# luisdiaz1997/GPzoo

Measured on AMD Instinct MI355X. Metric: ELBO evals/sec (L=32-latent evaluations, all GPUs) at M=2048 inducing, N=200000, L=32 latents/GPU x 1 GPU(s), higher is better.
Workload: dtype f32; 1 GPU; BASELINE configs[2]: Slide-seq-shaped synthetic, N=200000 spots, M=2048, L=32 latents/GPU x 1 GPU(s), matern32, f32; latents_total=32, whitened=True, chunk=0, factor_dtype=f64

## Files before the change

gpzoo_amd/csrc/gemmw.hip:

```cpp
#include "gemmw.h"

#include "cov.h"


#include <cmath>
#include <mutex>
#include <type_traits>
#include <utility>

#ifndef GPZ_W_ABL
#define GPZ_W_ABL 0
#endif

namespace gpz {

typedef float f32x4 __attribute__((ext_vector_type(4)));

enum { WB_MEM = 0, WB_GEN = 1 };
enum { WA_DENSE = 0, WA_LOWER = 1, WA_UPPER = 2 };
enum { WE_STORE_STATS = 0,
       WE_STATS = 1,
       WE_STORE = 2,
       WE_STORE_COLSCALE = 3,
       WE_WBAR = 4,
       WE_KBAR = 5,
       WE_ADD_COLSCALE = 6 };

struct WParams {
  const float* A; int64_t lda, sA0;
  const float* B; int64_t ldb, sB0;
  const float* Z; int64_t MD;
  const float* X; int64_t nreal;
  const float* sigma; const float* ell;
  float* C; int64_t ldc, sC0;
  const float* mu; int64_t sMu;
  float* ps_sq; float* ps_mu; int64_t ncols;
  const float* colscale; const float* colvec; int64_t sCs;
  const float* rowvec; int64_t sRv;
  const float* aux;
  int64_t M;
  int L, nblk, mtw, nt, W, strips;
  int pair, colmajor;
  const int32_t* gate;
};

constexpr int W_BK = 16;

template <int TM, int TN, int BSRC, int D>
struct WLds {
  static constexpr int A_ELEMS = TM * W_BK;
  static constexpr int RPP = 256 / TN;
  static constexpr int PITCH = 256 + (RPP == 2 ? 8 : RPP == 1 ? 4 : 16);
  static constexpr int B_ELEMS = (W_BK / RPP) * PITCH;
  static constexpr int STAGE = A_ELEMS + B_ELEMS;
  static constexpr int ZB = 128 * D;
  static constexpr size_t bytes = sizeof(float) * (2 * STAGE + (BSRC == WB_GEN ? 2 * ZB : 0));
};

template <int TM, int TN, int BSRC, int ATRI, int EPI, int KIND, int D>
__global__ __launch_bounds__(64 * (TM / 128) * (TN / 32)) __attribute__((amdgpu_waves_per_eu(4, 4))) void gemmw_kernel(const WParams p) {
  constexpr int BK = W_BK;
  if (p.gate && *p.gate == 0) return;
  constexpr int WMW = TM / 128, WNW = TN / 32;
  constexpr int NW = WMW * WNW;
  static_assert(NW == 8 || NW == 16, "8 or 16 waves of 128 x 32");
  using G = WLds<TM, TN, BSRC, D>;
  constexpr int RPP = G::RPP, PITCH = G::PITCH;
  extern __shared__ __attribute__((aligned(1024))) char smem_raw[];
  float* const smem = reinterpret_cast<float*>(smem_raw);
  auto sA = [&](int buf) -> float* { return smem + buf * G::STAGE; };
  auto sB = [&](int buf) -> float* { return smem + buf * G::STAGE + G::A_ELEMS; };
  float* const sZ = smem + 2 * G::STAGE;
  auto addrB = [](int k, int n) { return (k / RPP) * PITCH + (k % RPP) * TN + n; };

  int tj, b0, leg_ti[2], nlegs = 1;
  {
    const int bid = blockIdx.x;
    const int x = bid & 7, s = bid >> 3;
    if (BSRC == WB_GEN) {
      const int ug = s / p.W, within = s - ug * p.W;
      const int u = ug * 8 + x;
      const int per_level = p.L * p.strips;
      if (u >= p.mtw * per_level) return;
      const int level = u / per_level, rem = u - level * per_level;
      leg_ti[0] = leg_ti[1] = (ATRI == WA_LOWER) ? p.mtw - 1 - level : level;
      b0 = rem / p.strips;
      tj = (rem - b0 * p.strips) * p.W + within;
    } else {
      const int per_unit = (p.pair ? (p.mtw + 1) >> 1 : p.mtw) * p.W;
      const int u = (s / per_unit) * 8 + x, within = s % per_unit;
      if (u >= p.L * p.strips) return;
      b0 = u / p.strips;
      const int nrow = p.pair ? (p.mtw + 1) >> 1 : p.mtw;
      const int pi = p.colmajor ? within % nrow : within / p.W, far = p.pair ? p.mtw - 1 - pi : pi;
      const int strip = u - b0 * p.strips, c0 = strip * p.nt / p.strips, c1 = (strip + 1) * p.nt / p.strips;
      tj = c0 + (p.colmajor ? within / nrow : within % p.W);
      if (tj >= c1) return;
      const bool long_first = ((s >> 5) & 1) == 0;
      leg_ti[0] = ((ATRI == WA_LOWER) == long_first) ? far : pi;
      leg_ti[1] = ((ATRI == WA_LOWER) == long_first) ? pi : far;
      nlegs = far == pi ? 1 : 2;
      if (!p.pair) leg_ti[0] = leg_ti[1] = (ATRI == WA_LOWER) ? p.mtw - 1 - pi : pi;
    }
    if (tj >= p.nt) return;
  }
  const int tid = threadIdx.x, lane = tid & 63;
  const int wave = __builtin_amdgcn_readfirstlane(tid >> 6);
  const int wn = wave % WNW;
  const int r = lane & 15, q = lane >> 4;
  const int Mp = p.nblk * 128;

  typedef __attribute__((address_space(3))) void lds_void;
  constexpr int NPA = TM / (16 * NW);
#if defined(__HIP_DEVICE_COMPILE__)
  const __amdgpu_buffer_rsrc_t a_rsrc = __builtin_amdgcn_make_buffer_rsrc(
      const_cast<float*>(p.A + b0 * p.sA0), 0, (int)(p.lda * Mp * sizeof(float)), 0x00020000);
  const __amdgpu_buffer_rsrc_t b_rsrc = __builtin_amdgcn_make_buffer_rsrc(
      const_cast<float*>(BSRC == WB_MEM ? p.B + b0 * p.sB0 : p.Z), 0,
      (int)((BSRC == WB_MEM ? p.ldb * Mp : p.MD) * sizeof(float)), 0x00020000);
#endif
  auto k_begin_of = [&](int ti) { return (ATRI == WA_UPPER) ? TM * ti : 0; };
  auto k_end_of = [&](int ti) { return (ATRI == WA_LOWER) ? min(TM * (ti + 1), Mp) : Mp; };
  int a_soff[NPA], b_soff = 0;
  auto gperm = [](int w) { const int t = (w >> 2) & 3; return (((t >> 1) ^ t) & 1) << 1 | (t >> 1); };
  const int a_voff = ((lane >> 2) * (int)p.lda + (((lane & 3) ^ gperm(lane >> 2)) * 4)) * (int)sizeof(float);
  const int b_voff = ((lane / (TN / 4)) * (int)p.ldb + (lane % (TN / 4)) * 4) * (int)sizeof(float);
  bool abl_first = true;
  auto stage_load = [&](int buf) __attribute__((always_inline)) {
    if ((GPZ_W_ABL & 2) && !abl_first) return;
    abl_first = false;
#if defined(__HIP_DEVICE_COMPILE__)
#pragma unroll
    for (int h = 0; h < NPA; ++h) {
      __builtin_amdgcn_raw_ptr_buffer_load_lds(a_rsrc, (lds_void*)(sA(buf) + (NPA * wave + h) * 256), 16, a_voff, a_soff[h], 0, 0);
      a_soff[h] += BK * (int)sizeof(float);
    }
    if constexpr (BSRC == WB_MEM) {
      constexpr int NPB = (W_BK / RPP) / NW;
      static_assert(BSRC != WB_MEM || (NPB * NW * RPP == W_BK && NPB >= 1), "whole B pieces per wave");
#pragma unroll
      for (int h = 0; h < NPB; ++h)
        __builtin_amdgcn_raw_ptr_buffer_load_lds(b_rsrc, (lds_void*)(sB(buf) + (wave + NW * h) * PITCH), 16, b_voff,
                                                 b_soff + h * NW * RPP * (int)p.ldb * (int)sizeof(float), 0, 0);
      b_soff += BK * (int)p.ldb * (int)sizeof(float);
    }
#endif
  };
  auto tile_begin = [&](int ti) __attribute__((always_inline)) {
    const int kb = k_begin_of(ti);
#pragma unroll
    for (int h = 0; h < NPA; ++h) {
      int row = ti * TM + (NPA * wave + h) * 16;
      while (row >= Mp) row -= 128;
      a_soff[h] = (row * (int)p.lda + kb) * (int)sizeof(float);
    }
    b_soff = ((kb + RPP * wave) * (int)p.ldb + tj * TN) * (int)sizeof(float);
    stage_load(0);
  };

  constexpr int NXC = TN / 64;
  float xc[NXC][D], ampn[NXC], c0n[NXC], c2n[NXC];
  CovConst cc = {0.f, 0.f, 0.f, 0.f};
  if constexpr (BSRC == WB_GEN) {
    cc = cov_const<KIND>(p.sigma[b0], p.ell[b0]);
#pragma unroll
    for (int h = 0; h < NXC; ++h) {
      const int64_t n = (int64_t)tj * TN + h * 64 + lane;
      const bool real = n < p.nreal;
#pragma unroll
      for (int k = 0; k < D; ++k) xc[h][k] = real ? p.X[n * D + k] : 0.f;
      ampn[h] = real ? cc.amp : 0.f;
      c0n[h] = (KIND != 0 && !real) ? 0.f : cc.c0;
      c2n[h] = real ? cc.c2 : 0.f;
    }
  }
  auto z_load = [&](int blk) __attribute__((always_inline)) {
#if defined(__HIP_DEVICE_COMPILE__)
    if (wave < 2 * D)
      __builtin_amdgcn_raw_ptr_buffer_load_lds(b_rsrc, (lds_void*)(sZ + (blk & 1) * G::ZB + wave * 64), 4, lane * 4,
                                               (blk * G::ZB + wave * 64) * 4, 0, 0);
#endif
  };
  auto b_generate = [&](int buf, int step) __attribute__((always_inline)) {
#pragma unroll
    for (int i = 0; i < BK / NW; ++i) {
      const int kk = wave + NW * i, kg = step * BK + kk;
      const float* zp = sZ + ((kg >> 7) & 1) * G::ZB + (kg & 127) * D;
      float z[D];
#pragma unroll
      for (int k = 0; k < D; ++k) z[k] = zp[k];
#pragma unroll
      for (int h = 0; h < NXC; ++h) {
        const float v = (GPZ_W_ABL & 1) ? z[0] + xc[h][0]
                                        : cov_value<KIND>(cov_radial<KIND>(cov_d2<D>(z, xc[h])), ampn[h], c0n[h], cc.c1, c2n[h]);
        sB(buf)[addrB(kk, h * 64 + lane)] = v;
      }
    }
  };

  f32x4 acc[8][2];

  int wm = 0, nk = 0, db = 0, n_a = 0, fr_a = 0, step0 = 0, t = 0, next_ti = -1;
  bool active = false;
  int fr_b[4];
#pragma unroll
  for (int j = 0; j < 4; ++j) fr_b[j] = addrB(4 * q + j, wn * 32 + r);

  auto mma_step = [&](int buf, auto lo_c, auto hi_c) __attribute__((always_inline)) {
    constexpr int LO = decltype(lo_c)::value, HI = decltype(hi_c)::value;
    float bf[4][2];
#pragma unroll
    for (int j = 0; j < 4; ++j)
#pragma unroll
      for (int ni = 0; ni < 2; ++ni) bf[j][ni] = sB(buf)[fr_b[j] + ni * 16];
#pragma unroll
    for (int half = 0; half < 2; ++half) {
      f32x4 fa[4];
#pragma unroll
      for (int m = 0; m < 4; ++m)
        if (half * 4 + m >= LO && half * 4 + m <= HI)
          fa[m] = *reinterpret_cast<const f32x4*>(sA(buf) + fr_a + (half * 4 + m) * 16 * BK);
#pragma unroll
      for (int j = 0; j < 4; ++j)
#pragma unroll
        for (int m = 0; m < 4; ++m)
#pragma unroll
          for (int ni = 0; ni < 2; ++ni)
            if (half * 4 + m >= LO && half * 4 + m <= HI)
              acc[half * 4 + m][ni] = __builtin_amdgcn_mfma_f32_16x16x4f32(fa[m][j], bf[j][ni], acc[half * 4 + m][ni], 0, 0, 0);
    }
  };

  using std::integral_constant;
  auto step = [&](auto par_c, auto run_c, auto lo_c, auto hi_c) __attribute__((always_inline)) {
    constexpr int P = decltype(par_c)::value;
    if (t + 1 < nk) {
      stage_load(P ^ 1);
      if constexpr (BSRC == WB_GEN) {
        const int st = step0 + t;
        if ((st & 7) == 0 && (st >> 3) + 1 < p.nblk) z_load((st >> 3) + 1);
        b_generate(P ^ 1, st + 1);
      }
    } else if (next_ti >= 0) {
      tile_begin(next_ti);
    }
    if constexpr (decltype(run_c)::value) mma_step(P, lo_c, hi_c);
    if (GPZ_W_ABL & 16) {
      asm volatile("s_waitcnt lgkmcnt(0)" ::: "memory");
      __builtin_amdgcn_s_barrier();
    } else {
      asm volatile("s_waitcnt vmcnt(0)" ::: "memory");
      if (!(GPZ_W_ABL & 8)) __syncthreads();
    }
    ++t;
  };
  using no_run = integral_constant<bool, false>;
  using run = integral_constant<bool, true>;
  using i0 = integral_constant<int, 0>;
  using i1 = integral_constant<int, 1>;
  using i7 = integral_constant<int, 7>;
  auto idle_until = [&](int end) __attribute__((always_inline)) {
    while (t < end) { step(i0{}, no_run{}, i0{}, i7{}); step(i1{}, no_run{}, i0{}, i7{}); }
  };
  auto full_until = [&](int end) __attribute__((always_inline)) {
    while (t < end) { step(i0{}, run{}, i0{}, i7{}); step(i1{}, run{}, i0{}, i7{}); }
  };
  auto diagonal = [&](auto self, auto u_c) __attribute__((always_inline)) -> void {
    constexpr int U = decltype(u_c)::value;
    if constexpr (ATRI == WA_LOWER) step(integral_constant<int, U & 1>{}, run{}, integral_constant<int, U>{}, i7{});
    else step(integral_constant<int, U & 1>{}, run{}, i0{}, integral_constant<int, U>{});
    if constexpr (U + 1 < 8) self(self, integral_constant<int, U + 1>{});
  };

  tile_begin(leg_ti[0]);
#pragma unroll 1
  for (int leg = 0; leg < nlegs; ++leg) {
    const int ti = leg_ti[leg];
    wm = WMW == 1 ? 0 : (wave / WNW) ^ ((ti ^ tj) & 1);
    const int k_begin = k_begin_of(ti);
    nk = (k_end_of(ti) - k_begin) / BK;
    db = WMW * ti + wm;
    active = db < p.nblk && (int64_t)tj * TN + wn * 32 < p.ncols;
    n_a = 8 * (ATRI == WA_LOWER ? db : wm);
    fr_a = (wm * 128 + r) * BK + ((q ^ gperm(r)) * 4);
    step0 = k_begin / BK;
    t = 0;
    next_ti = leg + 1 < nlegs ? leg_ti[leg + 1] : -1;
#pragma unroll
    for (int mi = 0; mi < 8; ++mi)
#pragma unroll
      for (int ni = 0; ni < 2; ++ni) acc[mi][ni] = f32x4{0, 0, 0, 0};
    if constexpr (BSRC == WB_GEN) {
      z_load(step0 >> 3);
      asm volatile("s_waitcnt vmcnt(0)" ::: "memory");
      __syncthreads();
      b_generate(0, step0);
    }
    if (leg == 0) asm volatile("s_waitcnt vmcnt(0)" ::: "memory");
    asm volatile("s_waitcnt lgkmcnt(0)" ::: "memory");
    __builtin_amdgcn_s_barrier();
    if (!active) {
      idle_until(nk);
    } else if constexpr (ATRI == WA_DENSE) {
      full_until(nk);
    } else if constexpr (ATRI == WA_LOWER) {
      full_until(n_a);
      diagonal(diagonal, i0{});
      idle_until(nk);
    } else {
      idle_until(n_a);
      diagonal(diagonal, i0{});
      full_until(nk);
    }

    if (!active) continue;
    if (GPZ_W_ABL & 4) {
      float sum = 0.f;
#pragma unroll
      for (int mi = 0; mi < 8; ++mi)
#pragma unroll
        for (int ni = 0; ni < 2; ++ni)
#pragma unroll
          for (int g = 0; g < 4; ++g) sum += acc[mi][ni][g];
      if (sum == 12345.678f) p.ps_sq[0] = sum;
      continue;
    }
    const int64_t row0 = (int64_t)db * 128;
    const int64_t ccol0 = (int64_t)tj * TN + wn * 32;
    if (BSRC == WB_GEN && row0 + 128 > p.M) {
#pragma unroll
      for (int mi = 0; mi < 8; ++mi)
#pragma unroll
        for (int g = 0; g < 4; ++g)
          if (row0 + mi * 16 + 4 * q + g >= p.M) {
#pragma unroll
            for (int ni = 0; ni < 2; ++ni) acc[mi][ni][g] = 0.f;
          }
    }
    if constexpr (EPI == WE_STORE_STATS || EPI == WE_STATS) {
      float ssq[2] = {0.f, 0.f}, smu[2] = {0.f, 0.f};
#pragma unroll
      for (int mi = 0; mi < 8; ++mi) {
        f32x4 m4 = {0, 0, 0, 0};
        if constexpr (EPI == WE_STORE_STATS) m4 = *reinterpret_cast<const f32x4*>(p.mu + b0 * p.sMu + row0 + 4 * q + mi * 16);
#pragma unroll
        for (int g = 0; g < 4; ++g)
#pragma unroll
          for (int ni = 0; ni < 2; ++ni) {
            const float v = acc[mi][ni][g];
            ssq[ni] = __builtin_fmaf(v, v, ssq[ni]);
            if constexpr (EPI == WE_STORE_STATS) smu[ni] = __builtin_fmaf(m4[g], v, smu[ni]);
          }
      }
#pragma unroll
      for (int ni = 0; ni < 2; ++ni) {
        ssq[ni] += __shfl_xor(ssq[ni], 16); ssq[ni] += __shfl_xor(ssq[ni], 32);
        if constexpr (EPI == WE_STORE_STATS) { smu[ni] += __shfl_xor(smu[ni], 16); smu[ni] += __shfl_xor(smu[ni], 32); }
        if (q == 0) {
          const int64_t o = ((int64_t)b0 * p.nblk + db) * p.ncols + ccol0 + ni * 16 + r;
          p.ps_sq[o] = ssq[ni];
          if constexpr (EPI == WE_STORE_STATS) p.ps_mu[o] = smu[ni];
        }
      }
    }
    if constexpr (EPI != WE_STATS) {
      constexpr int LDE = 36;
      static_assert(NW * 16 * LDE <= G::STAGE, "the epilogue strips fit tile buffer 1");
      float* strip = sA(1) + wave * (16 * LDE);
      float* Cg = p.C + b0 * p.sC0 + row0 * p.ldc + ccol0;
      int srow = lane >> 3;
      asm volatile("" : "+v"(srow));
      const int c4 = (lane & 7) * 4;
      float cs[2] = {1.f, 1.f};
      if constexpr (EPI == WE_STORE_COLSCALE) {
#pragma unroll
        for (int ni = 0; ni < 2; ++ni) cs[ni] = p.colscale[b0 * p.sCs + ccol0 + ni * 16 + r];
      }
      f32x4 sc = {0, 0, 0, 0}, cv = {0, 0, 0, 0};
      if constexpr (EPI == WE_WBAR || EPI == WE_KBAR || EPI == WE_ADD_COLSCALE)
        sc = *reinterpret_cast<const f32x4*>(p.colscale + b0 * p.sCs + ccol0 + c4);
      if constexpr (EPI == WE_WBAR || EPI == WE_KBAR)
        cv = *reinterpret_cast<const f32x4*>(p.colvec + b0 * p.sCs + ccol0 + c4);
#pragma unroll
      for (int mi = 0; mi < 8; ++mi) {
#pragma unroll
        for (int ni = 0; ni < 2; ++ni)
#pragma unroll
          for (int g = 0; g < 4; ++g) strip[(4 * q + g) * LDE + ni * 16 + r] = cs[ni] * acc[mi][ni][g];
        __builtin_amdgcn_wave_barrier();
        f32x4 w[2];
        float rv[2];
        if constexpr (EPI == WE_WBAR || EPI == WE_KBAR || EPI == WE_ADD_COLSCALE) {
#pragma unroll
          for (int it = 0; it < 2; ++it) {
            const int64_t row = mi * 16 + it * 8 + srow;
            if constexpr (EPI == WE_WBAR) w[it] = *reinterpret_cast<const f32x4*>(p.aux + b0 * p.sC0 + (row0 + row) * p.ldc + ccol0 + c4);
            if constexpr (EPI == WE_ADD_COLSCALE) w[it] = *reinterpret_cast<const f32x4*>(Cg + (int64_t)row * p.ldc + c4);
            if constexpr (EPI != WE_ADD_COLSCALE) rv[it] = p.rowvec[b0 * p.sRv + row0 + row];
          }
        }
#pragma unroll
        for (int it = 0; it < 2; ++it) {
          const int row = it * 8 + srow;
          f32x4 v = *reinterpret_cast<const f32x4*>(strip + row * LDE + c4);
          if constexpr (EPI == WE_WBAR) {
#pragma unroll
            for (int e = 0; e < 4; ++e) v[e] = v[e] + rv[it] * cv[e] - w[it][e] * sc[e];
          }
          if constexpr (EPI == WE_KBAR) {
#pragma unroll
            for (int e = 0; e < 4; ++e) v[e] = v[e] * sc[e] + rv[it] * cv[e];
          }
          if constexpr (EPI == WE_ADD_COLSCALE) {
#pragma unroll
            for (int e = 0; e < 4; ++e) v[e] = w[it][e] + v[e] * sc[e];
          }
          *reinterpret_cast<f32x4*>(Cg + (int64_t)(mi * 16 + row) * p.ldc + c4) = v;
        }
        __builtin_amdgcn_wave_barrier();
      }
    }
  }
}

struct NTParams {
  const float* A; const float* B; float* C;
  int64_t ld, sAB, ldc, sC;
  int K, nblk, mt, L, T;
  int S, Ks;
  float* part; int64_t sPart;
  const float* w; int64_t sW;
  const int32_t* gate;
  const float* gm; float* vpart;
};

template <int TM, bool WTS>
__global__ __launch_bounds__(TM * 2) __attribute__((amdgpu_waves_per_eu(4, 4))) void gemmw_nt_kernel(const NTParams p) {
  constexpr int BK = W_BK, TN = 128;
  if (p.gate && *p.gate == 0) return;
  constexpr int NW = TM / 32;
  constexpr int A_ELEMS = TM * BK, B_ELEMS = TN * BK, STAGE = A_ELEMS + B_ELEMS;
  extern __shared__ __attribute__((aligned(1024))) char smem_raw[];
  float* const smem = reinterpret_cast<float*>(smem_raw);
  auto sA = [&](int buf) -> float* { return smem + buf * STAGE; };
  auto sB = [&](int buf) -> float* { return smem + buf * STAGE + A_ELEMS; };
  int b0, ti, tj, piece;
  {
    const int nb = (int)gridDim.x, qn = nb >> 3, rem = nb & 7, x = blockIdx.x & 7;
    const int lid0 = x * qn + min(x, rem) + (int)(blockIdx.x >> 3);
    const int grp = lid0 / p.T;
    const int t = lid0 - grp * p.T;
    b0 = grp / p.S;
    piece = grp - b0 * p.S;
    if constexpr (TM == 256) {
      int i = (int)((sqrtf(4.0f * (float)t + 1.0f) - 1.0f) * 0.5f);
      while ((i + 1) * (i + 2) <= t) ++i;
      while (i * (i + 1) > t) --i;
      ti = i; tj = t - i * (i + 1);
    } else {
      int i = (int)((sqrtf(8.0f * (float)t + 1.0f) - 1.0f) * 0.5f);
      while ((i + 1) * (i + 2) / 2 <= t) ++i;
      while (i * (i + 1) / 2 > t) --i;
      ti = i; tj = t - i * (i + 1) / 2;
    }
  }
  const int tid = threadIdx.x, lane = tid & 63;
  const int wave = __builtin_amdgcn_readfirstlane(tid >> 6);
  const int wm = wave >> 2, wn = wave & 3;
  const int r = lane & 15, q = lane >> 4;
  const int Mp = p.nblk * 128;
  const int db = (TM / 128) * ti + wm;
  const bool active = db < p.nblk && tj <= db;
  const bool same = TM == 128 && p.A == p.B && tj == ti;
  typedef __attribute__((address_space(3))) void lds_void;
#if defined(__HIP_DEVICE_COMPILE__)
  const __amdgpu_buffer_rsrc_t a_rsrc = __builtin_amdgcn_make_buffer_rsrc(
      const_cast<float*>(p.A + b0 * p.sAB), 0, (int)(p.ld * Mp * sizeof(float)), 0x00020000);
  const __amdgpu_buffer_rsrc_t b_rsrc = __builtin_amdgcn_make_buffer_rsrc(
      const_cast<float*>(p.B + b0 * p.sAB), 0, (int)(p.ld * Mp * sizeof(float)), 0x00020000);
#endif
  auto gperm = [](int w) { const int t = (w >> 2) & 3; return (((t >> 1) ^ t) & 1) << 1 | (t >> 1); };
  const int voff = ((lane >> 2) * (int)p.ld + (((lane & 3) ^ gperm(lane >> 2)) * 4)) * (int)sizeof(float);
  int a_soff[2], b_soff;
#pragma unroll
  for (int h = 0; h < 2; ++h) {
    int row = ti * TM + (2 * wave + h) * 16;
    while (row >= Mp) row -= 128;
    a_soff[h] = (row * (int)p.ld + piece * p.Ks) * (int)sizeof(float);
  }
  constexpr int NPB = 8 / NW;
  b_soff = ((tj * TN + wave * NPB * 16) * (int)p.ld + piece * p.Ks) * (int)sizeof(float);
  auto stage_load = [&](int buf) __attribute__((always_inline)) {
#if defined(__HIP_DEVICE_COMPILE__)
#pragma unroll
    for (int h = 0; h < 2; ++h) {
      __builtin_amdgcn_raw_ptr_buffer_load_lds(a_rsrc, (lds_void*)(sA(buf) + (2 * wave + h) * 256), 16, voff, a_soff[h], 0, 0);
      a_soff[h] += BK * (int)sizeof(float);
    }
    if (!same) {
#pragma unroll
      for (int h = 0; h < NPB; ++h)
        __builtin_amdgcn_raw_ptr_buffer_load_lds(b_rsrc, (lds_void*)(sB(buf) + (wave * NPB + h) * 256), 16, voff,
                                                 b_soff + h * 16 * (int)p.ld * (int)sizeof(float), 0, 0);
      b_soff += BK * (int)sizeof(float);
    }
#endif
  };
  const float* wk = WTS ? p.w + b0 * p.sW + (int64_t)piece * p.Ks + 4 * (lane >> 4) : nullptr;
  f32x4 wv;
  auto w_load = [&]() __attribute__((always_inline)) {
    if constexpr (WTS) { wv = *reinterpret_cast<const f32x4*>(wk); wk += BK; }
  };
  const int fr_a = (wm * 128 + r) * BK + ((q ^ gperm(r)) * 4);
  const int nk = (min(p.K, (piece + 1) * p.Ks) - piece * p.Ks) / BK;
  const bool split = p.S > 1;
  const bool diag = WTS && p.A == p.B && db == tj && db < p.nblk;
  if (diag) {
    auto diag_path = [&](auto wn_c) __attribute__((always_inline)) {
      constexpr int C0 = decltype(wn_c)::value, C1 = 7 - C0, N0 = 8 - C0, N1 = 8 - C1;
      const bool rd = p.gm != nullptr;
      const float* gk = rd ? p.gm + b0 * p.sW + (int64_t)piece * p.Ks + 4 * (lane >> 4) : nullptr;
      f32x4 gv = f32x4{0, 0, 0, 0};
      float pv0 = 0.f, pv1 = 0.f;
      f32x4 a0[N0], a1[N1];
#pragma unroll
      for (int i = 0; i < N0; ++i) a0[i] = f32x4{0, 0, 0, 0};
#pragma unroll
      for (int i = 0; i < N1; ++i) a1[i] = f32x4{0, 0, 0, 0};
      const int fb_off = r * BK + ((q ^ gperm(r)) * 4) + (same ? -A_ELEMS : 0);
      auto step = [&](int buf, bool more) __attribute__((always_inline)) {
        f32x4 f0 = *reinterpret_cast<const f32x4*>(sB(buf) + fb_off + C0 * 16 * BK);
        f32x4 f1 = *reinterpret_cast<const f32x4*>(sB(buf) + fb_off + C1 * 16 * BK);
        f0 *= wv; f1 *= wv;
        if (more) w_load();
#pragma unroll
        for (int mi = C0; mi < 8; ++mi) {
          const f32x4 fa = *reinterpret_cast<const f32x4*>(sA(buf) + fr_a + mi * 16 * BK);
#pragma unroll
          for (int j = 0; j < 4; ++j) {
            a0[mi - C0] = __builtin_amdgcn_mfma_f32_16x16x4f32(fa[j], f0[j], a0[mi - C0], 0, 0, 0);
            if (mi >= C1) a1[mi >= C1 ? mi - C1 : 0] = __builtin_amdgcn_mfma_f32_16x16x4f32(fa[j], f1[j], a1[mi >= C1 ? mi - C1 : 0], 0, 0, 0);
          }
          if (mi == 2 * C0 || mi == 2 * C0 + 1) {
            if (rd) {
              const f32x4 t = fa * gv;
              if (mi == 2 * C0) pv0 += (t[0] + t[1]) + (t[2] + t[3]); else pv1 += (t[0] + t[1]) + (t[2] + t[3]);
            }
          }
        }
        if (more && rd) { gv = *reinterpret_cast<const f32x4*>(gk); gk += BK; }
      };
      if (rd) { gv = *reinterpret_cast<const f32x4*>(gk); gk += BK; }
      stage_load(0);
      w_load();
      asm volatile("s_waitcnt vmcnt(0)" ::: "memory");
      __syncthreads();
      for (int t = 0; t < nk; t += 2) {
        if (t + 1 < nk) stage_load(1);
        step(0, t + 1 < nk);
        asm volatile("s_waitcnt vmcnt(0)" ::: "memory");
        __syncthreads();
        if (t + 2 < nk) stage_load(0);
        step(1, t + 2 < nk);
        asm volatile("s_waitcnt vmcnt(0)" ::: "memory");
        __syncthreads();
      }
      if (rd) {
        float* vp = p.vpart + ((int64_t)piece * p.L + b0) * Mp + db * 128;
        pv0 += __shfl_xor(pv0, 16); pv0 += __shfl_xor(pv0, 32);
        pv1 += __shfl_xor(pv1, 16); pv1 += __shfl_xor(pv1, 32);
        if (q == 0) { vp[(2 * C0) * 16 + r] = pv0; vp[(2 * C0 + 1) * 16 + r] = pv1; }
      }
      float* Cg = (split ? p.part + piece * p.sPart : p.C) + b0 * p.sC + (int64_t)db * 128 * p.ldc + (int64_t)tj * TN;
      auto put = [&](const f32x4& a, int mi, int c) __attribute__((always_inline)) {
        float* o = Cg + (int64_t)(mi * 16 + 4 * q) * p.ldc + c * 16 + r;
#pragma unroll
        for (int g = 0; g < 4; ++g) o[g * p.ldc] = split ? a[g] : o[g * p.ldc] + a[g];
      };
#pragma unroll
      for (int mi = C0; mi < 8; ++mi) put(a0[mi - C0], mi, C0);
#pragma unroll
      for (int mi = C1; mi < 8; ++mi) put(a1[mi - C1], mi, C1);
    };
    switch (wn) {
      case 0: diag_path(std::integral_constant<int, 0>{}); break;
      case 1: diag_path(std::integral_constant<int, 1>{}); break;
      case 2: diag_path(std::integral_constant<int, 2>{}); break;
      default: diag_path(std::integral_constant<int, 3>{}); break;
    }
    return;
  }
  f32x4 acc[8][2];
#pragma unroll
  for (int mi = 0; mi < 8; ++mi)
#pragma unroll
    for (int ni = 0; ni < 2; ++ni) acc[mi][ni] = f32x4{0, 0, 0, 0};
  const int fr_b = (wn * 32 + r) * BK + ((q ^ gperm(r)) * 4) + (same ? -A_ELEMS : 0);
  auto mma_step = [&](int buf, bool more) __attribute__((always_inline)) {
    f32x4 fb[2];
#pragma unroll
    for (int ni = 0; ni < 2; ++ni) {
      fb[ni] = *reinterpret_cast<const f32x4*>(sB(buf) + fr_b + ni * 16 * BK);
      if constexpr (WTS) fb[ni] *= wv;
    }
    if (more) w_load();
#pragma unroll
    for (int half = 0; half < 2; ++half) {
      f32x4 fa[4];
#pragma unroll
      for (int m = 0; m < 4; ++m) fa[m] = *reinterpret_cast<const f32x4*>(sA(buf) + fr_a + (half * 4 + m) * 16 * BK);
#pragma unroll
      for (int j = 0; j < 4; ++j)
#pragma unroll
        for (int m = 0; m < 4; ++m)
#pragma unroll
          for (int ni = 0; ni < 2; ++ni)
            acc[half * 4 + m][ni] = __builtin_amdgcn_mfma_f32_16x16x4f32(fa[m][j], fb[ni][j], acc[half * 4 + m][ni], 0, 0, 0);
    }
  };
  stage_load(0);
  w_load();
  asm volatile("s_waitcnt vmcnt(0)" ::: "memory");
  __syncthreads();
  if (active) {
    for (int t = 0; t < nk; t += 2) {
      if (t + 1 < nk) stage_load(1);
      mma_step(0, t + 1 < nk);
      asm volatile("s_waitcnt vmcnt(0)" ::: "memory");
      __syncthreads();
      if (t + 2 < nk) stage_load(0);
      mma_step(1, t + 2 < nk);
      asm volatile("s_waitcnt vmcnt(0)" ::: "memory");
      __syncthreads();
    }
  } else {
    for (int t = 0; t < nk; t += 2) {
      if (t + 1 < nk) stage_load(1);
      asm volatile("s_waitcnt vmcnt(0)" ::: "memory");
      __syncthreads();
      if (t + 2 < nk) stage_load(0);
      asm volatile("s_waitcnt vmcnt(0)" ::: "memory");
      __syncthreads();
    }
    return;
  }
  constexpr int LDE = 36;
  float* strip = smem + wave * (32 * LDE);
  float* Cg = (split ? p.part + piece * p.sPart : p.C) + b0 * p.sC + (int64_t)db * 128 * p.ldc + (int64_t)tj * TN + wn * 32;
  const int srow = lane >> 3, c4 = (lane & 7) * 4;
#pragma unroll
  for (int pass = 0; pass < 4; ++pass) {
#pragma unroll
    for (int mm = 0; mm < 2; ++mm)
#pragma unroll
      for (int ni = 0; ni < 2; ++ni)
#pragma unroll
        for (int g = 0; g < 4; ++g) strip[(mm * 16 + 4 * q + g) * LDE + ni * 16 + r] = acc[pass * 2 + mm][ni][g];
    __builtin_amdgcn_wave_barrier();
    f32x4 cin[4];
#pragma unroll
    for (int it = 0; it < 4; ++it)
      cin[it] = split ? f32x4{0, 0, 0, 0} : *reinterpret_cast<const f32x4*>(Cg + (int64_t)(pass * 32 + it * 8 + srow) * p.ldc + c4);
#pragma unroll
    for (int it = 0; it < 4; ++it) {
      const int row = it * 8 + srow;
      const f32x4 v = *reinterpret_cast<const f32x4*>(strip + row * LDE + c4);
      *reinterpret_cast<f32x4*>(Cg + (int64_t)(pass * 32 + row) * p.ldc + c4) = cin[it] + v;
    }
    __builtin_amdgcn_wave_barrier();
  }
}

__global__ __launch_bounds__(256) void nt_reduce_kernel(float* __restrict__ C, const float* __restrict__ part, int S, int64_t sPart,
                                                        int Mp, int64_t total4, const int32_t* __restrict__ gate, int sym) {
  const int64_t i4 = (int64_t)blockIdx.x * 256 + threadIdx.x;
  if (i4 >= total4 || (gate && *gate == 0)) return;
  const int64_t e = i4 * 4;
  const int col = (int)(e % Mp), row = (int)((e / Mp) % Mp);
  if ((col >> 7) > (row >> 7) || (sym && (col >> 4) > (row >> 4))) return;
  f32x4 v = *reinterpret_cast<const f32x4*>(C + e);
  for (int s = 0; s < S; ++s) v += *reinterpret_cast<const f32x4*>(part + s * sPart + e);
  *reinterpret_cast<f32x4*>(C + e) = v;
}

__global__ __launch_bounds__(256) void nt_vsum_kernel(const float* __restrict__ vpart, int S, int64_t LM, double* __restrict__ v,
                                                      int64_t Mp, int64_t v_stride) {
  const int64_t i = (int64_t)blockIdx.x * 256 + threadIdx.x;
  if (i >= LM) return;
  double t = 0.0;
  for (int s = 0; s < S; ++s) t += (double)vpart[s * LM + i];
  v[(i / Mp) * v_stride + i % Mp] = t;
}

template <typename K>
static int launch_wide(K kernel, size_t lds, const WParams& p, int64_t nblocks, hipStream_t s, int threads = 512) {
  struct Seen { const void* fn; int dev; };
  static Seen seen[64];
  static int n_seen = 0;
  static std::mutex mu;
  int dev = 0;
  GPZ_HIP_OK(hipGetDevice(&dev));
  if (lds > 64 * 1024) {
    const void* fn = reinterpret_cast<const void*>(kernel);
    std::lock_guard<std::mutex> lock(mu);
    bool have = false;
    for (int i = 0; i < n_seen; ++i) have = have || (seen[i].fn == fn && seen[i].dev == dev);
    if (!have) {
      GPZ_HIP_OK(hipFuncSetAttribute(fn, hipFuncAttributeMaxDynamicSharedMemorySize, (int)lds));
      if (n_seen < 64) seen[n_seen++] = Seen{fn, dev};
    }
  }
  GPZ_REQUIRE(nblocks > 0 && nblocks < (1ll << 31), "wide product: bad grid");
  hipLaunchKernelGGL(kernel, dim3((unsigned)nblocks), dim3((unsigned)threads), lds, s, p);
  GPZ_LAUNCH_OK();
  return 0;
}

bool fused1_supported(int dtype, int kind, int d) {
  return dtype == GPZ_F32 && (d == 1 || d == 2) &&
         (kind == GPZ_KERNEL_RBF || kind == GPZ_KERNEL_MATERN32 || kind == GPZ_KERNEL_MATERN12 || kind == GPZ_KERNEL_MATERN52);
}

int fused1_launch(const Fused1Args& a, hipStream_t s) {
  GPZ_REQUIRE(fused1_supported(GPZ_F32, a.kind, a.d), "fused stage 1: kind=%d d=%d unsupported", a.kind, a.d);
  GPZ_REQUIRE(a.Mp % 128 == 0 && a.ncp % 128 == 0 && a.Mp > 0 && a.ncp > 0 && a.L > 0, "fused stage 1: bad extents");
  GPZ_REQUIRE(a.Mp * a.Mp * 4 < (1ll << 31) && a.M * a.d * 4 < (1ll << 31), "fused stage 1: M too large");
  constexpr int TM = 512, TN = 128;
  WParams p = {};
  p.A = a.Linv; p.lda = a.Mp; p.sA0 = a.Mp * a.Mp;
  p.Z = a.Z; p.MD = a.M * a.d; p.M = a.M;
  p.X = a.X; p.nreal = a.nreal;
  p.sigma = a.sigma; p.ell = a.ell;
  p.C = a.Wt; p.ldc = a.ncp; p.sC0 = a.Mp * a.ncp;
  p.mu = a.muE; p.sMu = a.Mp;
  p.ps_sq = a.ps_sq; p.ps_mu = a.ps_mu; p.ncols = a.ncp;
  p.L = a.L; p.nblk = (int)(a.Mp / 128); p.mtw = (int)((a.Mp + TM - 1) / TM); p.nt = (int)(a.ncp / TN);
  int strips = (p.nt + 31) / 32;
  const int want = (32 + p.mtw * p.L - 1) / (p.mtw * p.L);
  if (strips < want) strips = want < p.nt ? want : p.nt;
  p.W = (p.nt + strips - 1) / strips;
  p.strips = (p.nt + p.W - 1) / p.W;
  const int64_t units = (int64_t)p.mtw * p.L * p.strips;
  const int64_t nblocks = (units + 7) / 8 * 8 * p.W;
#define GPZ_W1(KIND, D) return launch_wide(gemmw_kernel<TM, TN, WB_GEN, WA_LOWER, WE_STORE_STATS, KIND, D>, \
                                           WLds<TM, TN, WB_GEN, D>::bytes, p, nblocks, s, 1024)
  if (a.kind == GPZ_KERNEL_MATERN32) { if (a.d == 2) GPZ_W1(1, 2); GPZ_W1(1, 1); }
  if (a.kind == GPZ_KERNEL_MATERN12) { if (a.d == 2) GPZ_W1(4, 2); GPZ_W1(4, 1); }
  if (a.kind == GPZ_KERNEL_MATERN52) { if (a.d == 2) GPZ_W1(5, 2); GPZ_W1(5, 1); }
  if (a.d == 2) GPZ_W1(0, 2);
  GPZ_W1(0, 1);
#undef GPZ_W1
}

bool wide_product_supported(int64_t Mp, int64_t ncp) {
  return Mp % 128 == 0 && ncp % 128 == 0 && Mp * Mp * 4 < (1ll << 31) && Mp * ncp * 4 < (1ll << 31);
}

template <int TM, int TN>
static int wide_product_launch_t(const WideArgs& a, hipStream_t s) {
  WParams p = {};
  p.A = a.A; p.lda = a.Mp; p.sA0 = a.Mp * a.Mp;
  p.B = a.B; p.ldb = a.ncp; p.sB0 = a.Mp * a.ncp;
  p.C = a.C; p.ldc = a.ncp; p.sC0 = a.Mp * a.ncp;
  p.mu = a.mu; p.sMu = a.Mp;
  p.ps_sq = a.ps_sq; p.ps_mu = a.ps_mu; p.ncols = a.ncp; p.M = a.Mp;
  p.colscale = a.colscale; p.colvec = a.colvec; p.sCs = a.ncp; p.rowvec = a.rowvec; p.sRv = a.Mp; p.aux = a.aux;
  p.gate = a.gate;
  p.L = a.L; p.nblk = (int)(a.Mp / 128); p.mtw = (int)((a.Mp + TM - 1) / TM); p.nt = (int)((a.ncp + TN - 1) / TN);
  constexpr int WMAX = 4096 / TN;
  int strips = (p.nt + WMAX - 1) / WMAX;
  const int want = (8 + p.L - 1) / p.L;
  if (strips < want) strips = want < p.nt ? want : p.nt;
  p.strips = strips;
  p.W = (p.nt + strips - 1) / strips;
  const int64_t units = (int64_t)p.L * p.strips;
  const int64_t paired = (units + 7) / 8 * 8 * ((p.mtw + 1) / 2) * p.W;
  p.pair = p.colmajor = paired >= 4 * 512;
  const int64_t nblocks = p.pair ? paired : (units + 7) / 8 * 8 * p.mtw * p.W;
  constexpr size_t lds = WLds<TM, TN, WB_MEM, 1>::bytes;
#define GPZ_WM(ATRI, EPI) return launch_wide(gemmw_kernel<TM, TN, WB_MEM, ATRI, EPI, 0, 1>, lds, p, nblocks, s)
  switch (a.epilogue) {
    case WIDE_STORE_STATS:
      GPZ_REQUIRE(!a.upper && a.C && a.mu && a.ps_sq && a.ps_mu, "wide product: store + statistics is the lower-triangular product and needs C, mu and both slabs");
      GPZ_WM(WA_LOWER, WE_STORE_STATS);
    case WIDE_STATS:
      GPZ_REQUIRE(a.upper && a.ps_sq, "wide product: statistics only is the upper-triangular product");
      GPZ_WM(WA_UPPER, WE_STATS);
    case WIDE_STORE:
      GPZ_REQUIRE(a.upper && a.C, "wide product: the plain store is built for the upper-triangular product");
      GPZ_WM(WA_UPPER, WE_STORE);
    case WIDE_STORE_COLSCALE:
      GPZ_REQUIRE(a.upper && a.C && a.colscale, "wide product: the column-scaled store is the upper-triangular product and needs the factors");
      GPZ_WM(WA_UPPER, WE_STORE_COLSCALE);
    case WIDE_WBAR:
      GPZ_REQUIRE(!a.upper && a.C && a.colscale && a.colvec && a.rowvec && a.aux, "wide product: the W-bar epilogue needs its operands");
      GPZ_WM(WA_LOWER, WE_WBAR);
    case WIDE_KBAR:
      GPZ_REQUIRE(a.upper == 2 && a.C && a.colscale && a.colvec && a.rowvec, "wide product: the K-bar epilogue is the dense product and needs its vectors");
      GPZ_WM(WA_DENSE, WE_KBAR);
    case WIDE_ADD_COLSCALE:
      GPZ_REQUIRE(a.upper == 1 && a.C && a.colscale, "wide product: the accumulating column-scaled store is the upper-triangular product");
      GPZ_WM(WA_UPPER, WE_ADD_COLSCALE);
    default: break;
  }
#undef GPZ_WM
  GPZ_REQUIRE(false, "wide product: unknown epilogue %d", a.epilogue);
}

int wide_product_launch(const WideArgs& a, hipStream_t s) {
  GPZ_REQUIRE(wide_product_supported(a.Mp, a.ncp) && a.L > 0, "wide product: bad extents");
  return wide_product_launch_t<128, 256>(a, s);
}

bool wide_nt_supported(int64_t Mp, int64_t K) {
  return Mp % 128 == 0 && K % 128 == 0 && K > 0 && Mp * K * 4 < (1ll << 31);
}

static bool nt_small_tiles(int64_t nblk) { return nblk <= 4; }
static int64_t nt_tiles(int64_t nblk) {
  if (nt_small_tiles(nblk)) return nblk * (nblk + 1) / 2;
  const int64_t mt = (nblk + 1) / 2;
  return mt * (mt + 1) - (nblk & 1);
}

int wide_nt_pieces(int64_t Mp, int64_t K, int L) {
  const int64_t tiles = nt_tiles(Mp / 128) * L;
  if (tiles >= 384) {
    const double r = (double)tiles / 512.0;
    int best = 1;
    double best_cost = 1e30;
    for (int S = 1; S <= 4; ++S) {
      if (S > 1 && K / S < 2048) break;
      const double rounds = r * S, cost = std::ceil(rounds - 1e-9) / rounds * (1.0 + 0.015 * (S - 1));
      if (cost < best_cost - 1e-9) { best_cost = cost; best = S; }
    }
    return best;
  }
  int64_t S = (nt_small_tiles(Mp / 128) ? 1024 : 512) / tiles;
  S = std::min<int64_t>(S, K / 1024);
  S = std::min<int64_t>(S, 16);
  return (int)std::max<int64_t>(S, 1);
}

size_t wide_nt_vpart_floats(int64_t Mp, int64_t K, int L) { return (size_t)wide_nt_pieces(Mp, K, L) * L * Mp; }

size_t wide_nt_scratch_floats(int64_t Mp, int64_t K, int L) {
  const int S = wide_nt_pieces(Mp, K, L);
  return S > 1 ? (size_t)S * L * Mp * Mp : 0;
}

int wide_nt_launch(const float* A, const float* B, float* C, int64_t Mp, int64_t K, int L, hipStream_t s, float* scratch,
                   const float* w, const int32_t* gate, const float* gm, float* vpart, double* v, int64_t v_stride) {
  GPZ_REQUIRE(A && B && C && wide_nt_supported(Mp, K) && L > 0, "wide A B^T: bad arguments");
  GPZ_REQUIRE(!gm || (w && vpart && v && A == B), "wide A B^T: the row products A gm need weights, A == B and their buffers");
  NTParams p;
  p.w = w; p.sW = K; p.gate = gate; p.gm = gm; p.vpart = vpart;
  p.A = A; p.B = B; p.C = C; p.ld = K; p.sAB = Mp * K; p.ldc = Mp; p.sC = Mp * Mp;
  p.K = (int)K; p.nblk = (int)(Mp / 128); p.mt = (p.nblk + 1) / 2; p.L = L;
  const bool small = nt_small_tiles(p.nblk);
  p.T = (int)nt_tiles(p.nblk);
  int S = scratch ? wide_nt_pieces(Mp, K, L) : 1;
  p.Ks = (int)(((K + S - 1) / S + 31) / 32 * 32);
  S = (int)((K + p.Ks - 1) / p.Ks);
  p.S = S; p.part = scratch; p.sPart = (int64_t)L * Mp * Mp;
  const int64_t nblocks = (int64_t)p.T * L * S;
  GPZ_REQUIRE(nblocks > 0 && nblocks < (1ll << 31), "wide A B^T: bad grid");
  if (small) {
    constexpr size_t lds = sizeof(float) * 2 * (128 + 128) * W_BK;
    if (w) hipLaunchKernelGGL((gemmw_nt_kernel<128, true>), dim3((unsigned)nblocks), dim3(256), lds, s, p);
    else hipLaunchKernelGGL((gemmw_nt_kernel<128, false>), dim3((unsigned)nblocks), dim3(256), lds, s, p);
  } else {
    constexpr size_t lds = sizeof(float) * 2 * (256 + 128) * W_BK;
    if (w) hipLaunchKernelGGL((gemmw_nt_kernel<256, true>), dim3((unsigned)nblocks), dim3(512), lds, s, p);
    else hipLaunchKernelGGL((gemmw_nt_kernel<256, false>), dim3((unsigned)nblocks), dim3(512), lds, s, p);
  }
  GPZ_LAUNCH_OK();
  if (S > 1) {
    const int64_t total4 = (int64_t)L * Mp * Mp / 4;
    hipLaunchKernelGGL(nt_reduce_kernel, dim3((unsigned)((total4 + 255) / 256)), dim3(256), 0, s, C, scratch, S, p.sPart, (int)Mp, total4, gate, (int)(w != nullptr && A == B));
    GPZ_LAUNCH_OK();
  }
  if (gm) {
    const int64_t LM = (int64_t)L * Mp;
    hipLaunchKernelGGL(nt_vsum_kernel, dim3((unsigned)((LM + 255) / 256)), dim3(256), 0, s, vpart, S, LM, v, Mp, v_stride);
    GPZ_LAUNCH_OK();
  }
  return 0;
}

}
```

Baseline: 2.649 ELBO evals/s.

## Add symmetric 256x256 diagonal superblock tiles for weighted A A^T product

For the symmetric weighted NT product, the tile schedule is remapped so each diagonal 256x256 block runs as one superblock tile. In that tile all eight waves read a single A stage from LDS and compute only the lower-triangular 16x16 fragments, instead of splitting the diagonal into separate 128-row diagonal and off-diagonal tiles. This cuts redundant global loads and triangular waste on the diagonal and reduces the tile count, which also changes the split-K piece selection. It adds a new code path with heavier per-wave register use and unbalanced MFMA work across waves, plus an env-var fallback to the legacy path.

Measured after the change: 2.643 ELBO evals/s. No clear change (-0.2%).

```diff
diff --git a/gpzoo_amd/csrc/gemmw.hip b/gpzoo_amd/csrc/gemmw.hip
--- a/gpzoo_amd/csrc/gemmw.hip
+++ b/gpzoo_amd/csrc/gemmw.hip
@@ -3,7 +3,10 @@
 #include "cov.h"
 
 
+#include <algorithm>
 #include <cmath>
+#include <cstdlib>
+#include <cstring>
 #include <mutex>
 #include <type_traits>
 #include <utility>
@@ -432,6 +435,7 @@
   const float* w; int64_t sW;
   const int32_t* gate;
   const float* gm; float* vpart;
+  int sb;
 };
 
 template <int TM, bool WTS>
@@ -445,6 +449,7 @@
   auto sA = [&](int buf) -> float* { return smem + buf * STAGE; };
   auto sB = [&](int buf) -> float* { return smem + buf * STAGE + A_ELEMS; };
   int b0, ti, tj, piece;
+  bool sblock = false;
   {
     const int nb = (int)gridDim.x, qn = nb >> 3, rem = nb & 7, x = blockIdx.x & 7;
     const int lid0 = x * qn + min(x, rem) + (int)(blockIdx.x >> 3);
@@ -452,7 +457,19 @@
     const int t = lid0 - grp * p.T;
     b0 = grp / p.S;
     piece = grp - b0 * p.S;
-    if constexpr (TM == 256) {
+    if (TM == 256 && WTS && p.sb > 0) {
+      const int e2 = p.sb * p.sb;
+      if (t < e2) {
+        int i = (int)sqrtf((float)t);
+        while ((i + 1) * (i + 1) <= t) ++i;
+        while (i * i > t) --i;
+        ti = i;
+        sblock = t == i * i;
+        tj = sblock ? 2 * i : t - i * i - 1;
+      } else {
+        ti = p.sb; tj = t - e2;
+      }
+    } else if constexpr (TM == 256) {
       int i = (int)((sqrtf(4.0f * (float)t + 1.0f) - 1.0f) * 0.5f);
       while ((i + 1) * (i + 2) <= t) ++i;
       while (i * (i + 1) > t) --i;
@@ -514,6 +531,124 @@
   const int fr_a = (wm * 128 + r) * BK + ((q ^ gperm(r)) * 4);
   const int nk = (min(p.K, (piece + 1) * p.Ks) - piece * p.Ks) / BK;
   const bool split = p.S > 1;
+  if constexpr (TM == 256 && WTS) {
+    if (sblock) {
+      auto sb_path = [&](auto w_c) __attribute__((always_inline)) {
+        constexpr int C0 = decltype(w_c)::value, C1 = 15 - C0, N0 = 16 - C0, N1 = 16 - C1, GR = 2;
+        const bool rd = p.gm != nullptr;
+        const float* gk = (rd ? p.gm : p.w) + b0 * p.sW + (int64_t)piece * p.Ks;
+        const float* wks = p.w + b0 * p.sW + (int64_t)piece * p.Ks;
+        unsigned qo = 4 * (lane >> 4) * (unsigned)sizeof(float);
+        asm volatile("" : "+s"(gk), "+s"(wks), "+v"(qo));
+        f32x4 gv = f32x4{0, 0, 0, 0};
+        float pv0 = 0.f, pv1 = 0.f;
+        f32x4 a0[N0], a1[N1];
+#pragma unroll
+        for (int i = 0; i < N0; ++i) a0[i] = f32x4{0, 0, 0, 0};
+#pragma unroll
+        for (int i = 0; i < N1; ++i) a1[i] = f32x4{0, 0, 0, 0};
+        const int fr = r * BK + ((q ^ gperm(r)) * 4);
+        auto load_a = [&](int buf) __attribute__((always_inline)) {
+#if defined(__HIP_DEVICE_COMPILE__)
+#pragma unroll
+          for (int h = 0; h < 2; ++h) {
+            __builtin_amdgcn_raw_ptr_buffer_load_lds(a_rsrc, (lds_void*)(sA(buf) + (2 * wave + h) * 256), 16, voff, a_soff[h], 0, 0);
+            a_soff[h] += BK * (int)sizeof(float);
+          }
+#endif
+        };
+        auto step = [&](int buf, bool adv) __attribute__((always_inline)) {
+          f32x4 f0 = *reinterpret_cast<const f32x4*>(sA(buf) + fr + C0 * 16 * BK);
+          f32x4 f1 = *reinterpret_cast<const f32x4*>(sA(buf) + fr + C1 * 16 * BK);
+          f0 *= wv; f1 *= wv;
+          wv = *reinterpret_cast<const f32x4*>(reinterpret_cast<const char*>(wks) + qo);
+          wks += adv ? BK : 0;
+          f32x4 fa[2][GR];
+          auto fetch = [&](auto g_c) __attribute__((always_inline)) {
+            constexpr int G0 = decltype(g_c)::value, SL = ((G0 - C0) / GR) & 1;
+#pragma unroll
+            for (int m = 0; m < GR; ++m)
+              if (G0 + m < 16) fa[SL][m] = *reinterpret_cast<const f32x4*>(sA(buf) + fr + (G0 + m) * 16 * BK);
+          };
+          auto group = [&](auto self, auto g_c) __attribute__((always_inline)) -> void {
+            constexpr int G0 = decltype(g_c)::value, SL = ((G0 - C0) / GR) & 1;
+            if constexpr (G0 + GR < 16) fetch(std::integral_constant<int, G0 + GR>{});
+#pragma unroll
+            for (int j = 0; j < 4; ++j)
+#pragma unroll
+              for (int m = 0; m < GR; ++m) {
+                const int mi = G0 + m;
+                if (mi < 16) {
+                  a0[mi - C0] = __builtin_amdgcn_mfma_f32_16x16x4f32(fa[SL][m][j], f0[j], a0[mi - C0], 0, 0, 0);
+                  if (mi >= C1) a1[mi >= C1 ? mi - C1 : 0] = __builtin_amdgcn_mfma_f32_16x16x4f32(fa[SL][m][j], f1[j], a1[mi >= C1 ? mi - C1 : 0], 0, 0, 0);
+                }
+              }
+#pragma unroll
+            for (int m = 0; m < GR; ++m) {
+              const int mi = G0 + m;
+              if (mi == 2 * C0 || mi == 2 * C0 + 1) {
+                const f32x4 t = fa[SL][m] * gv;
+                if (mi == 2 * C0) pv0 += (t[0] + t[1]) + (t[2] + t[3]); else pv1 += (t[0] + t[1]) + (t[2] + t[3]);
+              }
+            }
+            __builtin_amdgcn_sched_barrier(0);
+            if constexpr (G0 + GR < 16) self(self, std::integral_constant<int, G0 + GR>{});
+          };
+          fetch(std::integral_constant<int, C0>{});
+          group(group, std::integral_constant<int, C0>{});
+          gv = *reinterpret_cast<const f32x4*>(reinterpret_cast<const char*>(gk) + qo);
+          gk += adv ? BK : 0;
+        };
+        gv = *reinterpret_cast<const f32x4*>(reinterpret_cast<const char*>(gk) + qo);
+        gk += nk > 1 ? BK : 0;
+        load_a(0);
+        wv = *reinterpret_cast<const f32x4*>(reinterpret_cast<const char*>(wks) + qo);
+        wks += nk > 1 ? BK : 0;
+        asm volatile("s_waitcnt vmcnt(0)" ::: "memory");
+        __syncthreads();
+        for (int t = 0; t < nk; t += 2) {
+          if (t + 1 < nk) load_a(1);
+          step(0, t + 2 < nk);
+          asm volatile("s_waitcnt vmcnt(0)" ::: "memory");
+          __syncthreads();
+          if (t + 2 < nk) load_a(0);
+          step(1, t + 3 < nk);
+          asm volatile("s_waitcnt vmcnt(0)" ::: "memory");
+          __syncthreads();
+        }
+        int tl = threadIdx.x;
+        asm volatile("" : "+v"(tl));
+        const int re = tl & 15, qe = (tl >> 4) & 3;
+        if (rd) {
+          float* vp = p.vpart + ((int64_t)piece * p.L + b0) * Mp + ti * 256;
+          pv0 += __shfl_xor(pv0, 16); pv0 += __shfl_xor(pv0, 32);
+          pv1 += __shfl_xor(pv1, 16); pv1 += __shfl_xor(pv1, 32);
+          if (qe == 0) { vp[(2 * C0) * 16 + re] = pv0; vp[(2 * C0 + 1) * 16 + re] = pv1; }
+        }
+        float* Cg = (split ? p.part + piece * p.sPart : p.C) + b0 * p.sC + (int64_t)ti * 256 * p.ldc + (int64_t)ti * 256;
+        auto put = [&](const f32x4& a, int mi, int c) __attribute__((always_inline)) {
+          float* o = Cg + (int64_t)(mi * 16 + 4 * qe) * p.ldc + c * 16 + re;
+#pragma unroll
+          for (int g = 0; g < 4; ++g) o[g * p.ldc] = split ? a[g] : o[g * p.ldc] + a[g];
+        };
+#pragma unroll
+        for (int mi = C0; mi < 16; ++mi) put(a0[mi - C0], mi, C0);
+#pragma unroll
+        for (int mi = C1; mi < 16; ++mi) put(a1[mi - C1], mi, C1);
+      };
+      switch (wave) {
+        case 0: sb_path(std::integral_constant<int, 0>{}); break;
+        case 1: sb_path(std::integral_constant<int, 1>{}); break;
+        case 2: sb_path(std::integral_constant<int, 2>{}); break;
+        case 3: sb_path(std::integral_constant<int, 3>{}); break;
+        case 4: sb_path(std::integral_constant<int, 4>{}); break;
+        case 5: sb_path(std::integral_constant<int, 5>{}); break;
+        case 6: sb_path(std::integral_constant<int, 6>{}); break;
+        default: sb_path(std::integral_constant<int, 7>{}); break;
+      }
+      return;
+    }
+  }
   const bool diag = WTS && p.A == p.B && db == tj && db < p.nblk;
   if (diag) {
     auto diag_path = [&](auto wn_c) __attribute__((always_inline)) {
@@ -817,14 +952,26 @@
 }
 
 static bool nt_small_tiles(int64_t nblk) { return nblk <= 4; }
-static int64_t nt_tiles(int64_t nblk) {
+static bool nt_legacy_diag() {
+  static const bool legacy = [] {
+    const char* e = getenv("GPZ_NT_DIAG");
+    return e && !strcmp(e, "legacy");
+  }();
+  return legacy;
+}
+static bool nt_superblocks(int64_t nblk, bool sym) { return sym && !nt_small_tiles(nblk) && !nt_legacy_diag(); }
+static int64_t nt_tiles(int64_t nblk, bool sym) {
   if (nt_small_tiles(nblk)) return nblk * (nblk + 1) / 2;
+  if (nt_superblocks(nblk, sym)) {
+    const int64_t e = nblk / 2;
+    return e * e + ((nblk & 1) ? nblk : 0);
+  }
   const int64_t mt = (nblk + 1) / 2;
   return mt * (mt + 1) - (nblk & 1);
 }
 
-int wide_nt_pieces(int64_t Mp, int64_t K, int L) {
-  const int64_t tiles = nt_tiles(Mp / 128) * L;
+static int nt_pieces(int64_t Mp, int64_t K, int L, bool sym) {
+  const int64_t tiles = nt_tiles(Mp / 128, sym) * L;
   if (tiles >= 384) {
     const double r = (double)tiles / 512.0;
     int best = 1;
@@ -841,6 +988,8 @@
   S = std::min<int64_t>(S, 16);
   return (int)std::max<int64_t>(S, 1);
 }
+
+int wide_nt_pieces(int64_t Mp, int64_t K, int L) { return std::max(nt_pieces(Mp, K, L, false), nt_pieces(Mp, K, L, true)); }
 
 size_t wide_nt_vpart_floats(int64_t Mp, int64_t K, int L) { return (size_t)wide_nt_pieces(Mp, K, L) * L * Mp; }
 
@@ -858,8 +1007,10 @@
   p.A = A; p.B = B; p.C = C; p.ld = K; p.sAB = Mp * K; p.ldc = Mp; p.sC = Mp * Mp;
   p.K = (int)K; p.nblk = (int)(Mp / 128); p.mt = (p.nblk + 1) / 2; p.L = L;
   const bool small = nt_small_tiles(p.nblk);
-  p.T = (int)nt_tiles(p.nblk);
-  int S = scratch ? wide_nt_pieces(Mp, K, L) : 1;
+  const bool sym = w != nullptr && A == B;
+  p.sb = nt_superblocks(p.nblk, sym) ? p.nblk / 2 : 0;
+  p.T = (int)nt_tiles(p.nblk, sym);
+  int S = scratch ? nt_pieces(Mp, K, L, sym) : 1;
   p.Ks = (int)(((K + S - 1) / S + 31) / 32 * 32);
   S = (int)((K + p.Ks - 1) / p.Ks);
   p.S = S; p.part = scratch; p.sPart = (int64_t)L * Mp * Mp;
```
